# Tencent/PocketFlow

Hardware: NVIDIA H100
Metric: images_per_sec_compression_aware_training_step (higher is better)
Workload: dtype f32

## Files before the change

pocketflow_b200/csrc/pf_nn.cu:

```cuda
#include <cstdlib>
#include <numeric>

#include "pf_common.cuh"

namespace {

constexpr int NT = 256;
constexpr int kColTile = 256;

struct ColTile {
  int c0, tc, nvec, nty, tx, ty;
  __device__ ColTile(int C) {
    c0 = blockIdx.x * kColTile;
    tc = min(kColTile, C - c0);
    nvec = tc >> 2;
    nty = NT / nvec;
    tx = threadIdx.x % nvec;
    ty = threadIdx.x / nvec;
  }
};

template <bool RANGE>
__global__ void __launch_bounds__(NT)
bn_stats_partial_kernel(const float* __restrict__ x, int M, int C, int rows_per_split,
                        float* __restrict__ part ) {
  __shared__ float sh[RANGE ? 4 : 2][NT * 4];
  constexpr int NF = RANGE ? 5 : 3;
  const ColTile t(C);
  const int r0 = blockIdx.y * rows_per_split;
  const int r1 = min(M, r0 + rows_per_split);
  const int col = t.c0 + t.tx * 4;
  float4 K = make_float4(0.f, 0.f, 0.f, 0.f), s1 = K, s2 = K;
  float4 mn = make_float4(INFINITY, INFINITY, INFINITY, INFINITY), mx = make_float4(-INFINITY, -INFINITY, -INFINITY, -INFINITY);
  if (t.ty < t.nty) {
    K = __ldg(reinterpret_cast<const float4*>(x + (size_t)r0 * C + col));
    auto acc = [&](const float4 v) {
      if (RANGE) {
        mn.x = fminf(mn.x, v.x); mn.y = fminf(mn.y, v.y); mn.z = fminf(mn.z, v.z); mn.w = fminf(mn.w, v.w);
        mx.x = fmaxf(mx.x, v.x); mx.y = fmaxf(mx.y, v.y); mx.z = fmaxf(mx.z, v.z); mx.w = fmaxf(mx.w, v.w);
      }
      const float dx = v.x - K.x, dy = v.y - K.y, dz = v.z - K.z, dw = v.w - K.w;
      s1.x += dx; s1.y += dy; s1.z += dz; s1.w += dw;
      s2.x = fmaf(dx, dx, s2.x); s2.y = fmaf(dy, dy, s2.y); s2.z = fmaf(dz, dz, s2.z); s2.w = fmaf(dw, dw, s2.w);
    };
    int r = r0 + t.ty;
    for (; r + 3 * t.nty < r1; r += 4 * t.nty) {
      const float4 v0 = pf_ld_stream(x + (size_t)r * C + col);
      const float4 v1 = pf_ld_stream(x + (size_t)(r + t.nty) * C + col);
      const float4 v2 = pf_ld_stream(x + (size_t)(r + 2 * t.nty) * C + col);
      const float4 v3 = pf_ld_stream(x + (size_t)(r + 3 * t.nty) * C + col);
      acc(v0); acc(v1); acc(v2); acc(v3);
    }
    for (; r < r1; r += t.nty) acc(pf_ld_stream(x + (size_t)r * C + col));
    float* a = &sh[0][(t.ty * t.nvec + t.tx) * 4];
    float* b = &sh[1][(t.ty * t.nvec + t.tx) * 4];
    a[0] = s1.x; a[1] = s1.y; a[2] = s1.z; a[3] = s1.w;
    b[0] = s2.x; b[1] = s2.y; b[2] = s2.z; b[3] = s2.w;
    if (RANGE) {
      float* lo = &sh[RANGE ? 2 : 0][(t.ty * t.nvec + t.tx) * 4];
      float* hi = &sh[RANGE ? 3 : 0][(t.ty * t.nvec + t.tx) * 4];
      lo[0] = mn.x; lo[1] = mn.y; lo[2] = mn.z; lo[3] = mn.w;
      hi[0] = mx.x; hi[1] = mx.y; hi[2] = mx.z; hi[3] = mx.w;
    }
  }
  __syncthreads();
  for (int c = threadIdx.x; c < t.tc; c += NT) {
    float a = 0.f, b = 0.f, lo = INFINITY, hi = -INFINITY;
    for (int y = 0; y < t.nty; ++y) {
      a += sh[0][(y * t.nvec + (c >> 2)) * 4 + (c & 3)];
      b += sh[1][(y * t.nvec + (c >> 2)) * 4 + (c & 3)];
      if (RANGE) {
        lo = fminf(lo, sh[RANGE ? 2 : 0][(y * t.nvec + (c >> 2)) * 4 + (c & 3)]);
        hi = fmaxf(hi, sh[RANGE ? 3 : 0][(y * t.nvec + (c >> 2)) * 4 + (c & 3)]);
      }
    }
    float* p = part + (size_t)blockIdx.y * NF * C;
    p[t.c0 + c] = __ldg(x + (size_t)r0 * C + t.c0 + c);
    p[C + t.c0 + c] = a;
    p[2 * C + t.c0 + c] = b;
    if (RANGE) {
      p[3 * C + t.c0 + c] = lo;
      p[4 * C + t.c0 + c] = hi;
    }
  }
}

constexpr int kFinalWarps = 4;
__global__ void __launch_bounds__(NT)
bn_stats_final_kernel(const float* __restrict__ part, int M, int C, int splits, int rows_per_split,
                      float eps, float momentum, float* __restrict__ mean, float* __restrict__ var,
                      float* __restrict__ rstd, float* __restrict__ mov_mean, float* __restrict__ mov_var,
                      int nf, const float* __restrict__ gamma, const float* __restrict__ beta, int act,
                      uint32_t* __restrict__ minmax_enc) {
  constexpr int CPB = NT / 32 / kFinalWarps;
  __shared__ double sh1[NT / 32], sh2[NT / 32];
  __shared__ float shlo[NT / 32], shhi[NT / 32];
  const int lane = threadIdx.x & 31, warp = threadIdx.x >> 5;
  const int cl = warp / kFinalWarps, sub = warp % kFinalWarps;
  const int c = blockIdx.x * CPB + cl;
  double S1 = 0.0, S2 = 0.0;
  float xlo = INFINITY, xhi = -INFINITY;
  const double K0 = c < C ? (double)part[c] : 0.0;
  if (c < C) {
    for (int s = sub * 32 + lane; s < splits; s += 32 * kFinalWarps) {
      const int r0 = s * rows_per_split;
      const double n = (double)(min(M, r0 + rows_per_split) - r0);
      const float* p = part + (size_t)s * nf * C;
      const double d = (double)p[c] - K0, s1 = p[C + c], s2 = p[2 * C + c];
      S1 += s1 + n * d;
      S2 += s2 + 2.0 * d * s1 + n * d * d;
      if (nf == 5) {
        xlo = fminf(xlo, p[3 * C + c]);
        xhi = fmaxf(xhi, p[4 * C + c]);
      }
    }
  }
// ... 110 lines not shown
      const float4 mu = __ldg(reinterpret_cast<const float4*>(mean + c));
      float4 rs = __ldg(reinterpret_cast<const float4*>(rstd + c));
      if (var_eps >= 0.f) {
        rs.x = __frsqrt_rn(__fadd_rn(rs.x, var_eps)); rs.y = __frsqrt_rn(__fadd_rn(rs.y, var_eps));
        rs.z = __frsqrt_rn(__fadd_rn(rs.z, var_eps)); rs.w = __frsqrt_rn(__fadd_rn(rs.w, var_eps));
      }
      const float4 ga = __ldg(reinterpret_cast<const float4*>(gamma + c));
      const float4 be = __ldg(reinterpret_cast<const float4*>(beta + c));
      apply4(pf_ld_stream(x + (i << 2)), mu, rs, ga, be, i);
      c += step;
      if (c >= (uint32_t)C) c -= (uint32_t)C;
    }
  }
  if (minmax_enc) {
    mn = pf_warp_min(mn);
    mx = pf_warp_max(mx);
    const int lane = threadIdx.x & 31, wid = threadIdx.x >> 5;
    if (lane == 0) { s_mn[wid] = mn; s_mx[wid] = mx; }
    __syncthreads();
    if (wid == 0) {
      mn = lane < NT / 32 ? s_mn[lane] : INFINITY;
      mx = lane < NT / 32 ? s_mx[lane] : -INFINITY;
      mn = pf_warp_min(mn);
      mx = pf_warp_max(mx);
      if (lane == 0 && mn <= mx) {
        atomicMin(minmax_enc, pf_enc(mn));
        atomicMax(minmax_enc + 1, pf_enc(mx));
      }
    }
  }
}

template <bool LEVELS_ONLY>
__global__ void __launch_bounds__(NT)
bn_apply_levels_kernel(const float* __restrict__ x, int64_t total, int C, int cshift, const float* __restrict__ mean,
                       const float* __restrict__ rstd, const float* __restrict__ gamma, const float* __restrict__ beta,
                       int act, float* __restrict__ y, void* __restrict__ p0, void* __restrict__ p1,
                       const uint32_t* __restrict__ q_range, int q_bits, pf_tc_act_hdr* __restrict__ hdr,
                       float* __restrict__ csum, int nseg) {
  const float qmn = pf_dec(__ldg(q_range)), qmx = pf_dec(__ldg(q_range + 1));
  const float q_alpha = __fadd_rn(__fsub_rn(qmx, qmn), 1e-10f), q_beta = qmn;
  const float q_k = pf_uq_kf(q_bits), q_ra = __frcp_rn(q_alpha), q_rk = __frcp_rn(q_k);
  const bool lev = q_bits <= 8 && q_beta == 0.f;
  if (blockIdx.x == 0 && threadIdx.x == 0) {
    hdr->scale = lev ? __fdiv_rn(q_alpha, q_k) : 1.f;
    hdr->nplanes = lev ? 1 : 2;
  }
  const int lane = threadIdx.x & 31;
  const int L = min(C >> 2, 32);
  const int64_t nvec = total >> 2;
  const int64_t stride = (int64_t)gridDim.x * NT;
  const int64_t first = (int64_t)blockIdx.x * NT + threadIdx.x;
  const uint32_t c = (uint32_t)((first << 2) & (int64_t)(C - 1));
  const float4 mu = __ldg(reinterpret_cast<const float4*>(mean + c));
  const float4 rs = __ldg(reinterpret_cast<const float4*>(rstd + c));
  const float4 ga = __ldg(reinterpret_cast<const float4*>(gamma + c));
  const float4 be = __ldg(reinterpret_cast<const float4*>(beta + c));
  auto emit = [&](float4 v, int64_t i, bool valid) {
    float4 lv;
    if (LEVELS_ONLY && lev) {
      lv.x = pf_quant_level(pf_bn_act(v.x, mu.x, rs.x, ga.x, be.x, act), q_alpha, q_beta, q_k, q_ra);
      lv.y = pf_quant_level(pf_bn_act(v.y, mu.y, rs.y, ga.y, be.y, act), q_alpha, q_beta, q_k, q_ra);
      lv.z = pf_quant_level(pf_bn_act(v.z, mu.z, rs.z, ga.z, be.z, act), q_alpha, q_beta, q_k, q_ra);
      lv.w = pf_quant_level(pf_bn_act(v.w, mu.w, rs.w, ga.w, be.w, act), q_alpha, q_beta, q_k, q_ra);
    } else {
      v.x = pf_fake_quant_lv(pf_bn_act(v.x, mu.x, rs.x, ga.x, be.x, act), q_alpha, q_beta, q_k, q_ra, q_rk, lv.x);
      v.y = pf_fake_quant_lv(pf_bn_act(v.y, mu.y, rs.y, ga.y, be.y, act), q_alpha, q_beta, q_k, q_ra, q_rk, lv.y);
// ... 181 lines not shown
  const float q_alpha = __fadd_rn(__fsub_rn(qmx, qmn), 1e-10f);
  const float q_k = pf_uq_kf(q_bits), q_ra = __frcp_rn(q_alpha);
  if (blockIdx.x == 0 && threadIdx.x == 0) {
    hdr->scale = qmn == 0.f ? __fdiv_rn(q_alpha, q_k) : 1.f;
    hdr->nplanes = qmn == 0.f ? 1 : 0;
  }
  const int64_t wbase = first - (lane >> 3);
  for (int64_t i = first; wbase + (i - first) < items; i += stride) {
    float part = 0.f;
    if (i < items && cok) {
      float y[16];
      load_bn(i, y);
      uint32_t w[4];
#pragma unroll
      for (int v = 0; v < 4; ++v) {
        const float l0 = pf_quant_level(y[4 * v], q_alpha, qmn, q_k, q_ra);
        const float l1 = pf_quant_level(y[4 * v + 1], q_alpha, qmn, q_k, q_ra);
        const float l2 = pf_quant_level(y[4 * v + 2], q_alpha, qmn, q_k, q_ra);
        const float l3 = pf_quant_level(y[4 * v + 3], q_alpha, qmn, q_k, q_ra);
        w[v] = (uint32_t)l0 | ((uint32_t)l1 << 8) | ((uint32_t)l2 << 16) | ((uint32_t)l3 << 24);
        part += (l0 + l1) + (l2 + l3);
      }
      uint2* dst = reinterpret_cast<uint2*>(levels + (i / nseg) * C + c0);
      dst[0] = make_uint2(w[0], w[1]);
      dst[1] = make_uint2(w[2], w[3]);
    }
    part += __shfl_xor_sync(0xffffffffu, part, 4);
    part += __shfl_xor_sync(0xffffffffu, part, 2);
    part += __shfl_xor_sync(0xffffffffu, part, 1);
    if (i < items && sub == 0) csum[i] = part;
  }
}

__global__ void __launch_bounds__(NT)
bn_bwd_partial_kernel(const float* __restrict__ dy, const float* __restrict__ x, int M, int C,
                      int rows_per_split, const float* __restrict__ mean, const float* __restrict__ rstd,
                      const float* __restrict__ gamma, const float* __restrict__ beta, int act,
                      float* __restrict__ part ) {
  __shared__ float sh[2][NT * 4];
  const ColTile t(C);
  const int r0 = blockIdx.y * rows_per_split;
  const int r1 = min(M, r0 + rows_per_split);
  const int col = t.c0 + t.tx * 4;
  float a[4] = {0.f, 0.f, 0.f, 0.f}, b[4] = {0.f, 0.f, 0.f, 0.f};
  if (t.ty < t.nty) {
    const float4 mu4 = __ldg(reinterpret_cast<const float4*>(mean + col));
    const float4 rs4 = __ldg(reinterpret_cast<const float4*>(rstd + col));
    const float4 ga4 = __ldg(reinterpret_cast<const float4*>(gamma + col));
    const float4 be4 = __ldg(reinterpret_cast<const float4*>(beta + col));
    const float mu[4] = {mu4.x, mu4.y, mu4.z, mu4.w}, rs[4] = {rs4.x, rs4.y, rs4.z, rs4.w};
    const float ga[4] = {ga4.x, ga4.y, ga4.z, ga4.w}, be[4] = {be4.x, be4.y, be4.z, be4.w};
    for (int r = r0 + t.ty; r < r1; r += t.nty) {
      const float4 d4 = pf_ld_stream(dy + (size_t)r * C + col);
      const float4 x4 = pf_ld_stream(x + (size_t)r * C + col);
      const float d[4] = {d4.x, d4.y, d4.z, d4.w}, xv[4] = {x4.x, x4.y, x4.z, x4.w};
#pragma unroll
      for (int j = 0; j < 4; ++j) {
        const float xh = __fmul_rn(__fsub_rn(xv[j], mu[j]), rs[j]);
        float dz = d[j];
        if (act) {
          const float z = __fadd_rn(__fmul_rn(xh, ga[j]), be[j]);
          if (!(z > 0.f) || (act == 2 && !(z < 6.f))) dz = 0.f;
        }
        a[j] += dz;
        b[j] = fmaf(dz, xh, b[j]);
      }
    }
    float* pa = &sh[0][(t.ty * t.nvec + t.tx) * 4];
    float* pb = &sh[1][(t.ty * t.nvec + t.tx) * 4];
#pragma unroll
    for (int j = 0; j < 4; ++j) { pa[j] = a[j]; pb[j] = b[j]; }
  }
  __syncthreads();
  for (int c = threadIdx.x; c < t.tc; c += NT) {
    float sa = 0.f, sb = 0.f;
    for (int y = 0; y < t.nty; ++y) {
      sa += sh[0][(y * t.nvec + (c >> 2)) * 4 + (c & 3)];
      sb += sh[1][(y * t.nvec + (c >> 2)) * 4 + (c & 3)];
    }
    float* p = part + (size_t)blockIdx.y * 2 * C;
    p[t.c0 + c] = sa;
    p[C + t.c0 + c] = sb;
  }
}

__global__ void __launch_bounds__(NT)
bn_bwd_final_kernel(const float* __restrict__ part, int C, int splits, float* __restrict__ dgamma,
                    float* __restrict__ dbeta) {
  constexpr int CPB = NT / 32 / kFinalWarps;
  __shared__ double sha[NT / 32], shb[NT / 32];
  const int lane = threadIdx.x & 31, warp = threadIdx.x >> 5;
  const int cl = warp / kFinalWarps, sub = warp % kFinalWarps;
  const int c = blockIdx.x * CPB + cl;
  double sa = 0.0, sb = 0.0;
  if (c < C) {
    for (int s = sub * 32 + lane; s < splits; s += 32 * kFinalWarps) {
      sa += part[(size_t)s * 2 * C + c];
      sb += part[(size_t)s * 2 * C + C + c];
    }
  }
#pragma unroll
  for (int o = 16; o > 0; o >>= 1) {
    sa += __shfl_down_sync(0xffffffffu, sa, o);
    sb += __shfl_down_sync(0xffffffffu, sb, o);
  }
  if (lane == 0) { sha[warp] = sa; shb[warp] = sb; }
  __syncthreads();
  if (c < C && sub == 0 && lane == 0) {
    for (int w = 1; w < kFinalWarps; ++w) { sa += sha[warp + w]; sb += shb[warp + w]; }
    dbeta[c] = (float)sa;
    dgamma[c] = (float)sb;
  }
}

__global__ void __launch_bounds__(NT)
bn_bwd_apply_kernel(const float* __restrict__ dy, const float* __restrict__ x, int64_t total, int C,
                    float inv_m, const float* __restrict__ mean, const float* __restrict__ rstd,
                    const float* __restrict__ gamma, const float* __restrict__ beta,
                    const float* __restrict__ dgamma, const float* __restrict__ dbeta, int act,
                    int accumulate, float* __restrict__ dx, void* __restrict__ dx_hi, void* __restrict__ dx_lo) {
  const int64_t nvec = total >> 2;
  const int64_t stride = (int64_t)gridDim.x * NT;
  int64_t i = (int64_t)blockIdx.x * NT + threadIdx.x;
  uint32_t c = (uint32_t)((i << 2) % (uint32_t)C);
  const uint32_t step = (uint32_t)((stride << 2) % (uint32_t)C);
  auto one = [&](const float4 d4, const float4 x4, const float4 mu4, const float4 rs4, const float4 ga4,
                 const float4 be4, const float4 dg4, const float4 db4, int64_t idx) {
    const float d[4] = {d4.x, d4.y, d4.z, d4.w}, xv[4] = {x4.x, x4.y, x4.z, x4.w};
    const float mu[4] = {mu4.x, mu4.y, mu4.z, mu4.w}, rs[4] = {rs4.x, rs4.y, rs4.z, rs4.w};
    const float ga[4] = {ga4.x, ga4.y, ga4.z, ga4.w}, be[4] = {be4.x, be4.y, be4.z, be4.w};
    const float dg[4] = {dg4.x, dg4.y, dg4.z, dg4.w}, db[4] = {db4.x, db4.y, db4.z, db4.w};
    float o[4];
#pragma unroll
    for (int j = 0; j < 4; ++j) {
      const float xh = __fmul_rn(__fsub_rn(xv[j], mu[j]), rs[j]);
      float dz = d[j];
      if (act) {
        const float z = __fadd_rn(__fmul_rn(xh, ga[j]), be[j]);
        if (!(z > 0.f) || (act == 2 && !(z < 6.f))) dz = 0.f;
      }
      o[j] = ga[j] * rs[j] * (dz - db[j] * inv_m - xh * dg[j] * inv_m);
    }
    float4 r = make_float4(o[0], o[1], o[2], o[3]);
    if (accumulate) {
      const float4 old = *reinterpret_cast<const float4*>(dx + (idx << 2));
      r.x += old.x; r.y += old.y; r.z += old.z; r.w += old.w;
    }
    if (dx) pf_st_stream(dx + (idx << 2), r);
    if (dx_hi) pf_st_planes4(dx_hi, dx_lo, idx << 2, r);
  };
  if (step == 0) {
    const float4 mu4 = __ldg(reinterpret_cast<const float4*>(mean + c)), rs4 = __ldg(reinterpret_cast<const float4*>(rstd + c));
    const float4 ga4 = __ldg(reinterpret_cast<const float4*>(gamma + c)), be4 = __ldg(reinterpret_cast<const float4*>(beta + c));
    const float4 dg4 = __ldg(reinterpret_cast<const float4*>(dgamma + c)), db4 = __ldg(reinterpret_cast<const float4*>(dbeta + c));
    for (; i + stride < nvec; i += 2 * stride) {
      const float4 d0 = pf_ld_stream(dy + (i << 2)), x0 = pf_ld_stream(x + (i << 2));
      const float4 d1 = pf_ld_stream(dy + ((i + stride) << 2)), x1 = pf_ld_stream(x + ((i + stride) << 2));
      one(d0, x0, mu4, rs4, ga4, be4, dg4, db4, i);
      one(d1, x1, mu4, rs4, ga4, be4, dg4, db4, i + stride);
    }
    for (; i < nvec; i += stride)
      one(pf_ld_stream(dy + (i << 2)), pf_ld_stream(x + (i << 2)), mu4, rs4, ga4, be4, dg4, db4, i);
  } else {
    for (; i < nvec; i += stride) {
      one(pf_ld_stream(dy + (i << 2)), pf_ld_stream(x + (i << 2)), __ldg(reinterpret_cast<const float4*>(mean + c)),
          __ldg(reinterpret_cast<const float4*>(rstd + c)), __ldg(reinterpret_cast<const float4*>(gamma + c)),
          __ldg(reinterpret_cast<const float4*>(beta + c)), __ldg(reinterpret_cast<const float4*>(dgamma + c)),
          __ldg(reinterpret_cast<const float4*>(dbeta + c)), i);
      c += step;
      if (c >= (uint32_t)C) c -= (uint32_t)C;
    }
  }
}

__global__ void __launch_bounds__(NT)
add_kernel(const float* __restrict__ a, const float* __restrict__ b, int64_t n, int accumulate,
           float* __restrict__ out) {
  const int64_t nvec = n >> 2;
  const int64_t stride = (int64_t)gridDim.x * NT;
  for (int64_t i = (int64_t)blockIdx.x * NT + threadIdx.x; i < nvec; i += stride) {
    float4 v = pf_ld4(a + (i << 2));
    if (b) {
      const float4 w = pf_ld4(b + (i << 2));
      v.x = __fadd_rn(v.x, w.x); v.y = __fadd_rn(v.y, w.y); v.z = __fadd_rn(v.z, w.z); v.w = __fadd_rn(v.w, w.w);
    }
    if (accumulate) {
      const float4 o = pf_ld4(out + (i << 2));
      v.x += o.x; v.y += o.y; v.z += o.z; v.w += o.w;
    }
    pf_st_stream(out + (i << 2), v);
  }
  if (blockIdx.x == 0 && threadIdx.x < (n & 3)) {
    const int64_t j = (nvec << 2) + threadIdx.x;
    float v = a[j] + (b ? b[j] : 0.f);
    out[j] = accumulate ? out[j] + v : v;
  }
}

// ... 217 lines not shown
__global__ void __launch_bounds__(NT)
softmax_fwd_kernel(const float* __restrict__ x, int n, int k, float* __restrict__ y) {
  const int lane = threadIdx.x & 31;
  const int row = blockIdx.x * (NT / 32) + (threadIdx.x >> 5);
  if (row >= n) return;
  const float* r = x + (size_t)row * k;
  float m = -INFINITY;
  for (int j = lane; j < k; j += 32) m = fmaxf(m, r[j]);
  m = pf_warp_max(m);
  float s = 0.f;
  for (int j = lane; j < k; j += 32) s += expf(r[j] - m);
  s = pf_warp_sum(s);
  for (int j = lane; j < k; j += 32) y[(size_t)row * k + j] = __fdiv_rn(expf(r[j] - m), s);
}
__global__ void __launch_bounds__(NT)
softmax_bwd_kernel(const float* __restrict__ dy, const float* __restrict__ y, int n, int k,
                   float* __restrict__ dx) {
  const int lane = threadIdx.x & 31;
  const int row = blockIdx.x * (NT / 32) + (threadIdx.x >> 5);
  if (row >= n) return;
  float dot = 0.f;
  for (int j = lane; j < k; j += 32) dot += dy[(size_t)row * k + j] * y[(size_t)row * k + j];
  dot = pf_warp_sum(dot);
  for (int j = lane; j < k; j += 32) {
    const size_t o = (size_t)row * k + j;
    dx[o] = (dy[o] - dot) * y[o];
  }
}

inline int bn_grid_cap() {
  const char* v = getenv("PF_BN_GRIDCAP");
  return (v && *v) ? atoi(v) : 8;
}
inline unsigned chan_grid(int64_t nvec, int C) {
  int64_t want = (nvec + NT - 1) / NT;
  const int64_t cap = (int64_t)PF_NUM_SMS * bn_grid_cap();
  if (want > cap) want = cap;
  if (want < 1) want = 1;
  const int c4 = C >> 2;
  int64_t mult = 1;
  while ((mult * NT) % c4 != 0 && mult < 64) mult <<= 1;
  if ((mult * NT) % c4 == 0) want = (want + mult - 1) / mult * mult;
  return (unsigned)want;
}

inline unsigned ew_grid(int64_t work_items) {
  int64_t want = (work_items + NT - 1) / NT;
  const int64_t cap = (int64_t)PF_NUM_SMS * 8;
  if (want < 1) want = 1;
  return (unsigned)(want < cap ? want : cap);
}

inline int bn_splits(int M, int C, int* rows_per_split) {
  const int col_tiles = (C + kColTile - 1) / kColTile;
  int splits = (8 * PF_NUM_SMS + col_tiles - 1) / col_tiles;
  const int max_by_rows = (M + 63) / 64;
  if (splits > max_by_rows) splits = max_by_rows;
  if (splits > PF_BN_MAX_SPLITS) splits = PF_BN_MAX_SPLITS;
  if (splits < 1) splits = 1;
  int rps = (M + splits - 1) / splits;
  *rows_per_split = rps;
  return (M + rps - 1) / rps;
}

__global__ void __launch_bounds__(NT)
fold_diag_blocks_kernel(const float* __restrict__ src, int g, int m, int n, float* __restrict__ dst) {
  const int i = blockIdx.x * NT + threadIdx.x;
  if (i >= m * n) return;
  const int r = i / n, c = i - r * n;
  float acc = 0.f;
  for (int b = 0; b < g; ++b) acc += src[(size_t)(b * m + r) * (g * n) + b * n + c];
  dst[i] = acc;
}
}

extern "C" {

int pf_bn_train_stats_range(const float* x_dev, int64_t m, int c, float eps, float momentum, float* mean_dev,
                            float* var_dev, float* rstd_dev, float* moving_mean_dev, float* moving_var_dev,
                            const float* gamma_dev, const float* beta_dev, int act, uint32_t* minmax_enc_dev,
                            float* ws_dev, void* stream) {
  PF_REQUIRE(m > 0 && c > 0 && m < (1ll << 31), "pf_bn_train_stats: bad shape");
  PF_REQUIRE((c & 3) == 0, "pf_bn_train_stats: C must be a multiple of 4 (got %d)", c);
  PF_REQUIRE(x_dev && mean_dev && var_dev && rstd_dev && ws_dev, "pf_bn_train_stats: null pointer");
  PF_REQUIRE((moving_mean_dev == nullptr) == (moving_var_dev == nullptr), "pf_bn_train_stats: moving stats come in pairs");
  PF_REQUIRE(minmax_enc_dev == nullptr || (gamma_dev && beta_dev && act >= 0 && act <= 2),
             "pf_bn_train_stats_range: the output range needs gamma, beta and act in {0,1,2}");
  int rps;
  const int splits = bn_splits((int)m, c, &rps);
  dim3 grid((c + kColTile - 1) / kColTile, splits);
  cudaStream_t st = (cudaStream_t)stream;
  const int nf = minmax_enc_dev ? 5 : 3;
  if (minmax_enc_dev) bn_stats_partial_kernel<true><<<grid, NT, 0, st>>>(x_dev, (int)m, c, rps, ws_dev);
  else bn_stats_partial_kernel<false><<<grid, NT, 0, st>>>(x_dev, (int)m, c, rps, ws_dev);
  PF_CHECK_LAUNCH("pf_bn_train_stats/partial");
  constexpr int kCPB = NT / 32 / kFinalWarps;
  bn_stats_final_kernel<<<(c + kCPB - 1) / kCPB, NT, 0, st>>>(ws_dev, (int)m, c, splits, rps, eps, momentum, mean_dev,
                                                         var_dev, rstd_dev, moving_mean_dev, moving_var_dev, nf, gamma_dev,
                                                         beta_dev, act, minmax_enc_dev);
  PF_CHECK_LAUNCH("pf_bn_train_stats/final");
  return PF_OK;
}

int pf_bn_train_stats(const float* x_dev, int64_t m, int c, float eps, float momentum, float* mean_dev,
                      float* var_dev, float* rstd_dev, float* moving_mean_dev, float* moving_var_dev,
                      float* ws_dev, void* stream) {
  return pf_bn_train_stats_range(x_dev, m, c, eps, momentum, mean_dev, var_dev, rstd_dev, moving_mean_dev, moving_var_dev,
                                 nullptr, nullptr, 0, nullptr, ws_dev, stream);
}

int pf_bn_eval_prepare(const float* moving_var_dev, int c, float eps, float* rstd_dev, void* stream) {
  PF_REQUIRE(c > 0 && moving_var_dev && rstd_dev, "pf_bn_eval_prepare: bad arguments");
  bn_eval_prepare_kernel<<<(c + NT - 1) / NT, NT, 0, (cudaStream_t)stream>>>(moving_var_dev, c, eps, rstd_dev);
  PF_CHECK_LAUNCH("pf_bn_eval_prepare");
  return PF_OK;
}

static int bn_apply_impl(const float* x_dev, int64_t m, int c, const float* mean_dev, const float* rstd_dev,
                         const float* gamma_dev, const float* beta_dev, int act, float* y_dev, void* y_hi_dev,
                         void* y_lo_dev, uint32_t* minmax_enc_dev, const uint32_t* q_range_dev, int q_bits, void* stream,
                         float var_eps = -1.f, const float* res_dev = nullptr) {
  PF_REQUIRE(m > 0 && c > 0 && (c & 3) == 0, "pf_bn_apply: bad shape (C must be a multiple of 4)");
  PF_REQUIRE(act >= 0 && act <= 2, "pf_bn_apply: act must be 0 (none), 1 (relu) or 2 (relu6)");
  PF_REQUIRE(x_dev && mean_dev && rstd_dev && gamma_dev && beta_dev, "pf_bn_apply: null pointer");
  PF_REQUIRE(y_dev || y_hi_dev, "pf_bn_apply: no output");
  PF_REQUIRE((y_hi_dev == nullptr) == (y_lo_dev == nullptr), "pf_bn_apply: planes come in pairs");
  PF_REQUIRE((((uintptr_t)y_hi_dev | (uintptr_t)y_lo_dev) & 7) == 0, "pf_bn_apply: planes must be 8-byte aligned");
// ... 20 lines not shown

int pf_bn_apply_eval(const float* x_dev, int64_t m, int c, const float* moving_mean_dev, const float* moving_var_dev,
                     float eps, const float* gamma_dev, const float* beta_dev, int act, float* y_dev, void* y_hi_dev,
                     void* y_lo_dev, uint32_t* minmax_enc_dev, void* stream) {
  PF_REQUIRE(eps >= 0.f, "pf_bn_apply_eval: eps < 0");
  return bn_apply_impl(x_dev, m, c, moving_mean_dev, moving_var_dev, gamma_dev, beta_dev, act, y_dev, y_hi_dev, y_lo_dev,
                       minmax_enc_dev, nullptr, 0, stream, eps);
}

int pf_bn_apply_quant(const float* x_dev, int64_t m, int c, const float* mean_dev, const float* rstd_dev,
                      const float* gamma_dev, const float* beta_dev, int act, const uint32_t* range_enc_dev, int bits,
                      float* y_dev, void* y_hi_dev, void* y_lo_dev, void* stream) {
  PF_REQUIRE(range_enc_dev != nullptr, "pf_bn_apply_quant: null range");
  PF_REQUIRE(bits >= 1 && bits <= 32, "pf_bn_apply_quant: bits must be in [1, 32]");
  return bn_apply_impl(x_dev, m, c, mean_dev, rstd_dev, gamma_dev, beta_dev, act, y_dev, y_hi_dev, y_lo_dev, nullptr,
                       range_enc_dev, bits, stream);
}

int pf_bn_apply_quant_levels(const float* x_dev, int64_t m, int c, const float* mean_dev, const float* rstd_dev,
                             const float* gamma_dev, const float* beta_dev, int act, const uint32_t* range_enc_dev,
                             int bits, float* y_dev, void* plane0_dev, void* plane1_dev, pf_tc_act_hdr* hdr_dev,
                             float* csum_dev, void* stream) {
  PF_REQUIRE(m > 0 && c >= 16 && (c & (c - 1)) == 0, "pf_bn_apply_quant_levels: C must be a power of two >= 16 (got %d)", c);
  PF_REQUIRE(act >= 0 && act <= 2, "pf_bn_apply_quant_levels: act must be 0 (none), 1 (relu) or 2 (relu6)");
  PF_REQUIRE(bits >= 1 && bits <= 32, "pf_bn_apply_quant_levels: bits must be in [1, 32]");
  PF_REQUIRE(x_dev && mean_dev && rstd_dev && gamma_dev && beta_dev && range_enc_dev && plane0_dev && plane1_dev && hdr_dev &&
                 csum_dev, "pf_bn_apply_quant_levels: null pointer");
  PF_REQUIRE((((uintptr_t)plane0_dev | (uintptr_t)plane1_dev | (uintptr_t)hdr_dev) & 7) == 0,
             "pf_bn_apply_quant_levels: planes / header must be 8-byte aligned");
  const int64_t total = m * c;
  int cshift = 0;
  while ((1 << cshift) < c) ++cshift;
  const int nseg = (c + 127) / 128;
  unsigned grid = chan_grid(total >> 2, c);
  PF_REQUIRE(((int64_t)grid * NT) % (c >> 2) == 0, "pf_bn_apply_quant_levels: C = %d too large for the channel-stationary grid", c);
  if (y_dev == nullptr && bits <= 8)
    bn_apply_levels_kernel<true><<<grid, NT, 0, (cudaStream_t)stream>>>(x_dev, total, c, cshift, mean_dev, rstd_dev, gamma_dev,
                                                                       beta_dev, act, nullptr, plane0_dev, plane1_dev,
                                                                       range_enc_dev, bits, hdr_dev, csum_dev, nseg);
  else
    bn_apply_levels_kernel<false><<<grid, NT, 0, (cudaStream_t)stream>>>(x_dev, total, c, cshift, mean_dev, rstd_dev, gamma_dev,
                                                                        beta_dev, act, y_dev, plane0_dev, plane1_dev,
                                                                        range_enc_dev, bits, hdr_dev, csum_dev, nseg);
  PF_CHECK_LAUNCH("pf_bn_apply_quant_levels");
  return PF_OK;
}

int pf_bn_eval_levels_u8(const float* x_dev, int64_t m, int c, const float* moving_mean_dev, const float* moving_var_dev,
                         float eps, const float* gamma_dev, const float* beta_dev, int act, int bits,
                         uint32_t* range_enc_dev, int have_range, void* levels_dev, pf_tc_act_hdr* hdr_dev,
                         float* csum_dev, void* stream) {
  const char* who = "pf_bn_eval_levels_u8";
  PF_REQUIRE(m > 0 && c >= 16 && c % 16 == 0, "%s: C must be a multiple of 16 (got %d)", who, c);
  PF_REQUIRE(act >= 0 && act <= 2, "%s: act must be 0 (none), 1 (relu) or 2 (relu6)", who);
  PF_REQUIRE(bits >= 1 && bits <= 8, "%s: u8 levels need 1..8 bits", who);
  PF_REQUIRE(eps >= 0.f, "%s: eps < 0", who);
  PF_REQUIRE(x_dev && moving_mean_dev && moving_var_dev && gamma_dev && beta_dev && range_enc_dev && levels_dev && hdr_dev &&
                 csum_dev, "%s: null pointer", who);
  PF_REQUIRE((((uintptr_t)x_dev | (uintptr_t)moving_mean_dev | (uintptr_t)moving_var_dev | (uintptr_t)gamma_dev |
               (uintptr_t)beta_dev) & 15) == 0 && (((uintptr_t)levels_dev | (uintptr_t)hdr_dev) & 7) == 0,
             "%s: fp32 tensors must be 16-byte aligned, levels / header 8-byte aligned", who);
  const int64_t total = m * c;
  const int nseg = (c + 127) / 128;
  cudaStream_t st = (cudaStream_t)stream;
  uint8_t* lv = reinterpret_cast<uint8_t*>(levels_dev);
  if (c & (c - 1)) {
    const int64_t items = m * nseg;
// ... 44 lines not shown

int pf_bn_apply_add_eval(const float* x_dev, int64_t m, int c, const float* moving_mean_dev, const float* moving_var_dev,
                         float eps, const float* gamma_dev, const float* beta_dev, const float* res_dev, float* y_dev,
                         void* y_hi_dev, void* y_lo_dev, void* stream) {
  PF_REQUIRE(eps >= 0.f, "pf_bn_apply_add_eval: eps < 0");
  PF_REQUIRE(res_dev != nullptr, "pf_bn_apply_add_eval: null residual");
  PF_REQUIRE((((uintptr_t)res_dev | (uintptr_t)x_dev | (uintptr_t)y_dev) & 15) == 0,
             "pf_bn_apply_add_eval: fp32 tensors must be 16-byte aligned");
  return bn_apply_impl(x_dev, m, c, moving_mean_dev, moving_var_dev, gamma_dev, beta_dev, 0, y_dev, y_hi_dev, y_lo_dev, nullptr,
                       nullptr, 0, stream, eps, res_dev);
}

int pf_bn_apply(const float* x_dev, int64_t m, int c, const float* mean_dev, const float* rstd_dev,
                const float* gamma_dev, const float* beta_dev, int act, float* y_dev,
                uint32_t* minmax_enc_dev, void* stream) {
  PF_REQUIRE(y_dev != nullptr, "pf_bn_apply: null pointer");
  return pf_bn_apply_planes(x_dev, m, c, mean_dev, rstd_dev, gamma_dev, beta_dev, act, y_dev, nullptr, nullptr,
                            minmax_enc_dev, stream);
}

int pf_bn_bwd_planes(const float* dy_dev, const float* x_dev, int64_t m, int c, const float* mean_dev,
                     const float* rstd_dev, const float* gamma_dev, const float* beta_dev, int act,
                     float* dgamma_dev, float* dbeta_dev, float* dx_dev, int accumulate, void* dx_hi_dev,
                     void* dx_lo_dev, float* ws_dev, void* stream) {
  PF_REQUIRE(m > 0 && c > 0 && (c & 3) == 0 && m < (1ll << 31), "pf_bn_bwd: bad shape (C must be a multiple of 4)");
  PF_REQUIRE(dy_dev && x_dev && mean_dev && rstd_dev && gamma_dev && beta_dev && dgamma_dev && dbeta_dev && ws_dev,
             "pf_bn_bwd: null pointer");
  PF_REQUIRE(dx_dev || dx_hi_dev, "pf_bn_bwd: no output");
  PF_REQUIRE((dx_hi_dev == nullptr) == (dx_lo_dev == nullptr), "pf_bn_bwd: planes come in pairs");
  PF_REQUIRE(!accumulate || dx_dev, "pf_bn_bwd: accumulate needs the fp32 dx");
  PF_REQUIRE((((uintptr_t)dx_hi_dev | (uintptr_t)dx_lo_dev) & 7) == 0, "pf_bn_bwd: planes must be 8-byte aligned");
  int rps;
  const int splits = bn_splits((int)m, c, &rps);
  dim3 grid((c + kColTile - 1) / kColTile, splits);
  cudaStream_t st = (cudaStream_t)stream;
  bn_bwd_partial_kernel<<<grid, NT, 0, st>>>(dy_dev, x_dev, (int)m, c, rps, mean_dev, rstd_dev, gamma_dev, beta_dev,
                                            act, ws_dev);
  PF_CHECK_LAUNCH("pf_bn_bwd/partial");
  bn_bwd_final_kernel<<<(c + NT / 32 / kFinalWarps - 1) / (NT / 32 / kFinalWarps), NT, 0, st>>>(ws_dev, c, splits, dgamma_dev, dbeta_dev);
  PF_CHECK_LAUNCH("pf_bn_bwd/final");
  const int64_t total = m * c;
  bn_bwd_apply_kernel<<<chan_grid(total >> 2, c), NT, 0, st>>>(dy_dev, x_dev, total, c, 1.f / (float)m, mean_dev, rstd_dev,
                                                        gamma_dev, beta_dev, dgamma_dev, dbeta_dev, act, accumulate,
                                                        dx_dev, dx_hi_dev, dx_lo_dev);
  PF_CHECK_LAUNCH("pf_bn_bwd/apply");
  return PF_OK;
}

int pf_bn_bwd(const float* dy_dev, const float* x_dev, int64_t m, int c, const float* mean_dev,
              const float* rstd_dev, const float* gamma_dev, const float* beta_dev, int act,
              float* dgamma_dev, float* dbeta_dev, float* dx_dev, int accumulate, float* ws_dev,
              void* stream) {
  PF_REQUIRE(dx_dev != nullptr, "pf_bn_bwd: null pointer");
  return pf_bn_bwd_planes(dy_dev, x_dev, m, c, mean_dev, rstd_dev, gamma_dev, beta_dev, act, dgamma_dev, dbeta_dev,
                          dx_dev, accumulate, nullptr, nullptr, ws_dev, stream);
}

int pf_fold_diag_blocks(const float* src_dev, int g, int m, int n, float* dst_dev, void* stream) {
  PF_REQUIRE(g >= 1 && m >= 1 && n >= 1 && (int64_t)m * n < (1ll << 30), "pf_fold_diag_blocks: bad shape");
  PF_REQUIRE(src_dev && dst_dev, "pf_fold_diag_blocks: null pointer");
  fold_diag_blocks_kernel<<<(m * n + NT - 1) / NT, NT, 0, (cudaStream_t)stream>>>(src_dev, g, m, n, dst_dev);
  PF_CHECK_LAUNCH("pf_fold_diag_blocks");
  return PF_OK;
}

int pf_add(const float* a_dev, const float* b_dev, int64_t n, int accumulate, float* out_dev, void* stream) {
  PF_REQUIRE(n >= 0, "pf_add: n < 0");
  if (n == 0) return PF_OK;
  PF_REQUIRE(a_dev && out_dev, "pf_add: null pointer");
  PF_REQUIRE((((uintptr_t)a_dev | (uintptr_t)b_dev | (uintptr_t)out_dev) & 15) == 0, "pf_add: 16-byte alignment required");
  add_kernel<<<ew_grid(n >> 2), NT, 0, (cudaStream_t)stream>>>(a_dev, b_dev, n, accumulate, out_dev);
  PF_CHECK_LAUNCH("pf_add");
  return PF_OK;
}

// ... 87 lines not shown
```

Baseline: 2749.

## Cap batchnorm grids to SM residency and make partial kernels loop over splits

The BN stats and backward partial kernels become grid-stride over row splits, with the grid capped to a per-SM CTA target and splits walked in reverse. Launch-bound minimum-block hints are added, and the backward partial loop is unrolled four rows at a time. The backward apply kernel goes from two to four vectors per iteration and loads the old dx before computing. The aim is to cut tail and wave-quantisation effects and expose more memory-level parallelism, at the cost of register pressure from the launch bounds and fewer CTAs for small shapes.

```diff
diff --git a/pocketflow_b200/csrc/pf_nn.cu b/pocketflow_b200/csrc/pf_nn.cu
--- a/pocketflow_b200/csrc/pf_nn.cu
+++ b/pocketflow_b200/csrc/pf_nn.cu
@@ -1,3 +1,4 @@
+#include <algorithm>
 #include <cstdlib>
 #include <numeric>
 
@@ -7,6 +8,10 @@
 
 constexpr int NT = 256;
 constexpr int kColTile = 256;
+constexpr int kStatsCtasPerSm = 4;
+constexpr int kBwdCtasPerSm = 3;
+constexpr int kBwdApplyCtasPerSm = 2;
+constexpr int kApplyLevelsCtasPerSm = 4;
 
 struct ColTile {
   int c0, tc, nvec, nty, tx, ty;
@@ -21,67 +26,71 @@
 };
 
 template <bool RANGE>
-__global__ void __launch_bounds__(NT)
-bn_stats_partial_kernel(const float* __restrict__ x, int M, int C, int rows_per_split,
+__global__ void __launch_bounds__(NT, kStatsCtasPerSm)
+bn_stats_partial_kernel(const float* __restrict__ x, int M, int C, int rows_per_split, int splits,
                         float* __restrict__ part ) {
   __shared__ float sh[RANGE ? 4 : 2][NT * 4];
   constexpr int NF = RANGE ? 5 : 3;
   const ColTile t(C);
-  const int r0 = blockIdx.y * rows_per_split;
-  const int r1 = min(M, r0 + rows_per_split);
   const int col = t.c0 + t.tx * 4;
-  float4 K = make_float4(0.f, 0.f, 0.f, 0.f), s1 = K, s2 = K;
-  float4 mn = make_float4(INFINITY, INFINITY, INFINITY, INFINITY), mx = make_float4(-INFINITY, -INFINITY, -INFINITY, -INFINITY);
-  if (t.ty < t.nty) {
-    K = __ldg(reinterpret_cast<const float4*>(x + (size_t)r0 * C + col));
-    auto acc = [&](const float4 v) {
+  for (int k = blockIdx.y; k < splits; k += gridDim.y) {
+    const int split = splits - 1 - k;
+    const int r0 = split * rows_per_split;
+    const int r1 = min(M, r0 + rows_per_split);
+    float4 K = make_float4(0.f, 0.f, 0.f, 0.f), s1 = K, s2 = K;
+    float4 mn = make_float4(INFINITY, INFINITY, INFINITY, INFINITY), mx = make_float4(-INFINITY, -INFINITY, -INFINITY, -INFINITY);
+    if (t.ty < t.nty) {
+      K = __ldg(reinterpret_cast<const float4*>(x + (size_t)r0 * C + col));
+      auto acc = [&](const float4 v) {
+        if (RANGE) {
+          mn.x = fminf(mn.x, v.x); mn.y = fminf(mn.y, v.y); mn.z = fminf(mn.z, v.z); mn.w = fminf(mn.w, v.w);
+          mx.x = fmaxf(mx.x, v.x); mx.y = fmaxf(mx.y, v.y); mx.z = fmaxf(mx.z, v.z); mx.w = fmaxf(mx.w, v.w);
+        }
+        const float dx = v.x - K.x, dy = v.y - K.y, dz = v.z - K.z, dw = v.w - K.w;
+        s1.x += dx; s1.y += dy; s1.z += dz; s1.w += dw;
+        s2.x = fmaf(dx, dx, s2.x); s2.y = fmaf(dy, dy, s2.y); s2.z = fmaf(dz, dz, s2.z); s2.w = fmaf(dw, dw, s2.w);
+      };
+      int r = r0 + t.ty;
+      for (; r + 3 * t.nty < r1; r += 4 * t.nty) {
+        const float4 v0 = pf_ld_stream(x + (size_t)r * C + col);
+        const float4 v1 = pf_ld_stream(x + (size_t)(r + t.nty) * C + col);
+        const float4 v2 = pf_ld_stream(x + (size_t)(r + 2 * t.nty) * C + col);
+        const float4 v3 = pf_ld_stream(x + (size_t)(r + 3 * t.nty) * C + col);
+        acc(v0); acc(v1); acc(v2); acc(v3);
+      }
+      for (; r < r1; r += t.nty) acc(pf_ld_stream(x + (size_t)r * C + col));
+      float* a = &sh[0][(t.ty * t.nvec + t.tx) * 4];
+      float* b = &sh[1][(t.ty * t.nvec + t.tx) * 4];
+      a[0] = s1.x; a[1] = s1.y; a[2] = s1.z; a[3] = s1.w;
+      b[0] = s2.x; b[1] = s2.y; b[2] = s2.z; b[3] = s2.w;
       if (RANGE) {
-        mn.x = fminf(mn.x, v.x); mn.y = fminf(mn.y, v.y); mn.z = fminf(mn.z, v.z); mn.w = fminf(mn.w, v.w);
-        mx.x = fmaxf(mx.x, v.x); mx.y = fmaxf(mx.y, v.y); mx.z = fmaxf(mx.z, v.z); mx.w = fmaxf(mx.w, v.w);
-      }
-      const float dx = v.x - K.x, dy = v.y - K.y, dz = v.z - K.z, dw = v.w - K.w;
-      s1.x += dx; s1.y += dy; s1.z += dz; s1.w += dw;
-      s2.x = fmaf(dx, dx, s2.x); s2.y = fmaf(dy, dy, s2.y); s2.z = fmaf(dz, dz, s2.z); s2.w = fmaf(dw, dw, s2.w);
-    };
-    int r = r0 + t.ty;
-    for (; r + 3 * t.nty < r1; r += 4 * t.nty) {
-      const float4 v0 = pf_ld_stream(x + (size_t)r * C + col);
-      const float4 v1 = pf_ld_stream(x + (size_t)(r + t.nty) * C + col);
-      const float4 v2 = pf_ld_stream(x + (size_t)(r + 2 * t.nty) * C + col);
-      const float4 v3 = pf_ld_stream(x + (size_t)(r + 3 * t.nty) * C + col);
-      acc(v0); acc(v1); acc(v2); acc(v3);
-    }
-    for (; r < r1; r += t.nty) acc(pf_ld_stream(x + (size_t)r * C + col));
-    float* a = &sh[0][(t.ty * t.nvec + t.tx) * 4];
-    float* b = &sh[1][(t.ty * t.nvec + t.tx) * 4];
-    a[0] = s1.x; a[1] = s1.y; a[2] = s1.z; a[3] = s1.w;
-    b[0] = s2.x; b[1] = s2.y; b[2] = s2.z; b[3] = s2.w;
-    if (RANGE) {
-      float* lo = &sh[RANGE ? 2 : 0][(t.ty * t.nvec + t.tx) * 4];
-      float* hi = &sh[RANGE ? 3 : 0][(t.ty * t.nvec + t.tx) * 4];
-      lo[0] = mn.x; lo[1] = mn.y; lo[2] = mn.z; lo[3] = mn.w;
-      hi[0] = mx.x; hi[1] = mx.y; hi[2] = mx.z; hi[3] = mx.w;
-    }
-  }
-  __syncthreads();
-  for (int c = threadIdx.x; c < t.tc; c += NT) {
-    float a = 0.f, b = 0.f, lo = INFINITY, hi = -INFINITY;
-    for (int y = 0; y < t.nty; ++y) {
-      a += sh[0][(y * t.nvec + (c >> 2)) * 4 + (c & 3)];
-      b += sh[1][(y * t.nvec + (c >> 2)) * 4 + (c & 3)];
+        float* lo = &sh[RANGE ? 2 : 0][(t.ty * t.nvec + t.tx) * 4];
+        float* hi = &sh[RANGE ? 3 : 0][(t.ty * t.nvec + t.tx) * 4];
+        lo[0] = mn.x; lo[1] = mn.y; lo[2] = mn.z; lo[3] = mn.w;
+        hi[0] = mx.x; hi[1] = mx.y; hi[2] = mx.z; hi[3] = mx.w;
+      }
+    }
+    __syncthreads();
+    for (int c = threadIdx.x; c < t.tc; c += NT) {
+      float a = 0.f, b = 0.f, lo = INFINITY, hi = -INFINITY;
+      for (int y = 0; y < t.nty; ++y) {
+        a += sh[0][(y * t.nvec + (c >> 2)) * 4 + (c & 3)];
+        b += sh[1][(y * t.nvec + (c >> 2)) * 4 + (c & 3)];
+        if (RANGE) {
+          lo = fminf(lo, sh[RANGE ? 2 : 0][(y * t.nvec + (c >> 2)) * 4 + (c & 3)]);
+          hi = fmaxf(hi, sh[RANGE ? 3 : 0][(y * t.nvec + (c >> 2)) * 4 + (c & 3)]);
+        }
+      }
+      float* p = part + (size_t)split * NF * C;
+      p[t.c0 + c] = __ldg(x + (size_t)r0 * C + t.c0 + c);
+      p[C + t.c0 + c] = a;
+      p[2 * C + t.c0 + c] = b;
       if (RANGE) {
-        lo = fminf(lo, sh[RANGE ? 2 : 0][(y * t.nvec + (c >> 2)) * 4 + (c & 3)]);
-        hi = fmaxf(hi, sh[RANGE ? 3 : 0][(y * t.nvec + (c >> 2)) * 4 + (c & 3)]);
-      }
-    }
-    float* p = part + (size_t)blockIdx.y * NF * C;
-    p[t.c0 + c] = __ldg(x + (size_t)r0 * C + t.c0 + c);
-    p[C + t.c0 + c] = a;
-    p[2 * C + t.c0 + c] = b;
-    if (RANGE) {
-      p[3 * C + t.c0 + c] = lo;
-      p[4 * C + t.c0 + c] = hi;
-    }
+        p[3 * C + t.c0 + c] = lo;
+        p[4 * C + t.c0 + c] = hi;
+      }
+    }
+    __syncthreads();
   }
 }
 
@@ -258,7 +267,7 @@
 }
 
 template <bool LEVELS_ONLY>
-__global__ void __launch_bounds__(NT)
+__global__ void __launch_bounds__(NT, kApplyLevelsCtasPerSm)
 bn_apply_levels_kernel(const float* __restrict__ x, int64_t total, int C, int cshift, const float* __restrict__ mean,
                        const float* __restrict__ rstd, const float* __restrict__ gamma, const float* __restrict__ beta,
                        int act, float* __restrict__ y, void* __restrict__ p0, void* __restrict__ p1,
@@ -506,55 +515,74 @@
   }
 }
 
-__global__ void __launch_bounds__(NT)
+__global__ void __launch_bounds__(NT, kBwdCtasPerSm)
 bn_bwd_partial_kernel(const float* __restrict__ dy, const float* __restrict__ x, int M, int C,
-                      int rows_per_split, const float* __restrict__ mean, const float* __restrict__ rstd,
+                      int rows_per_split, int splits, const float* __restrict__ mean, const float* __restrict__ rstd,
                       const float* __restrict__ gamma, const float* __restrict__ beta, int act,
                       float* __restrict__ part ) {
   __shared__ float sh[2][NT * 4];
   const ColTile t(C);
-  const int r0 = blockIdx.y * rows_per_split;
-  const int r1 = min(M, r0 + rows_per_split);
   const int col = t.c0 + t.tx * 4;
-  float a[4] = {0.f, 0.f, 0.f, 0.f}, b[4] = {0.f, 0.f, 0.f, 0.f};
+  float mu[4], rs[4], ga[4], be[4];
   if (t.ty < t.nty) {
     const float4 mu4 = __ldg(reinterpret_cast<const float4*>(mean + col));
     const float4 rs4 = __ldg(reinterpret_cast<const float4*>(rstd + col));
     const float4 ga4 = __ldg(reinterpret_cast<const float4*>(gamma + col));
     const float4 be4 = __ldg(reinterpret_cast<const float4*>(beta + col));
-    const float mu[4] = {mu4.x, mu4.y, mu4.z, mu4.w}, rs[4] = {rs4.x, rs4.y, rs4.z, rs4.w};
-    const float ga[4] = {ga4.x, ga4.y, ga4.z, ga4.w}, be[4] = {be4.x, be4.y, be4.z, be4.w};
-    for (int r = r0 + t.ty; r < r1; r += t.nty) {
-      const float4 d4 = pf_ld_stream(dy + (size_t)r * C + col);
-      const float4 x4 = pf_ld_stream(x + (size_t)r * C + col);
-      const float d[4] = {d4.x, d4.y, d4.z, d4.w}, xv[4] = {x4.x, x4.y, x4.z, x4.w};
-#pragma unroll
-      for (int j = 0; j < 4; ++j) {
-        const float xh = __fmul_rn(__fsub_rn(xv[j], mu[j]), rs[j]);
-        float dz = d[j];
-        if (act) {
-          const float z = __fadd_rn(__fmul_rn(xh, ga[j]), be[j]);
-          if (!(z > 0.f) || (act == 2 && !(z < 6.f))) dz = 0.f;
+    mu[0] = mu4.x; mu[1] = mu4.y; mu[2] = mu4.z; mu[3] = mu4.w;
+    rs[0] = rs4.x; rs[1] = rs4.y; rs[2] = rs4.z; rs[3] = rs4.w;
+    ga[0] = ga4.x; ga[1] = ga4.y; ga[2] = ga4.z; ga[3] = ga4.w;
+    be[0] = be4.x; be[1] = be4.y; be[2] = be4.z; be[3] = be4.w;
+  }
+  for (int k = blockIdx.y; k < splits; k += gridDim.y) {
+    const int split = splits - 1 - k;
+    const int r0 = split * rows_per_split;
+    const int r1 = min(M, r0 + rows_per_split);
+    float a[4] = {0.f, 0.f, 0.f, 0.f}, b[4] = {0.f, 0.f, 0.f, 0.f};
+    if (t.ty < t.nty) {
+      auto acc = [&](const float4 d4, const float4 x4) {
+        const float d[4] = {d4.x, d4.y, d4.z, d4.w}, xv[4] = {x4.x, x4.y, x4.z, x4.w};
+#pragma unroll
+        for (int j = 0; j < 4; ++j) {
+          const float xh = __fmul_rn(__fsub_rn(xv[j], mu[j]), rs[j]);
+          float dz = d[j];
+          if (act) {
+            const float z = __fadd_rn(__fmul_rn(xh, ga[j]), be[j]);
+            if (!(z > 0.f) || (act == 2 && !(z < 6.f))) dz = 0.f;
+          }
+          a[j] += dz;
+          b[j] = fmaf(dz, xh, b[j]);
         }
-        a[j] += dz;
-        b[j] = fmaf(dz, xh, b[j]);
-      }
-    }
-    float* pa = &sh[0][(t.ty * t.nvec + t.tx) * 4];
-    float* pb = &sh[1][(t.ty * t.nvec + t.tx) * 4];
-#pragma unroll
-    for (int j = 0; j < 4; ++j) { pa[j] = a[j]; pb[j] = b[j]; }
-  }
-  __syncthreads();
-  for (int c = threadIdx.x; c < t.tc; c += NT) {
-    float sa = 0.f, sb = 0.f;
-    for (int y = 0; y < t.nty; ++y) {
-      sa += sh[0][(y * t.nvec + (c >> 2)) * 4 + (c & 3)];
-      sb += sh[1][(y * t.nvec + (c >> 2)) * 4 + (c & 3)];
-    }
-    float* p = part + (size_t)blockIdx.y * 2 * C;
-    p[t.c0 + c] = sa;
-    p[C + t.c0 + c] = sb;
+      };
+      int r = r0 + t.ty;
+      for (; r + 3 * t.nty < r1; r += 4 * t.nty) {
+        const float* pd = dy + (size_t)r * C + col;
+        const float* px = x + (size_t)r * C + col;
+        const size_t rs1 = (size_t)t.nty * C;
+        const float4 d0 = pf_ld_stream(pd), x0 = pf_ld_stream(px);
+        const float4 d1 = pf_ld_stream(pd + rs1), x1 = pf_ld_stream(px + rs1);
+        const float4 d2 = pf_ld_stream(pd + 2 * rs1), x2 = pf_ld_stream(px + 2 * rs1);
+        const float4 d3 = pf_ld_stream(pd + 3 * rs1), x3 = pf_ld_stream(px + 3 * rs1);
+        acc(d0, x0); acc(d1, x1); acc(d2, x2); acc(d3, x3);
+      }
+      for (; r < r1; r += t.nty) acc(pf_ld_stream(dy + (size_t)r * C + col), pf_ld_stream(x + (size_t)r * C + col));
+      float* pa = &sh[0][(t.ty * t.nvec + t.tx) * 4];
+      float* pb = &sh[1][(t.ty * t.nvec + t.tx) * 4];
+#pragma unroll
+      for (int j = 0; j < 4; ++j) { pa[j] = a[j]; pb[j] = b[j]; }
+    }
+    __syncthreads();
+    for (int c = threadIdx.x; c < t.tc; c += NT) {
+      float sa = 0.f, sb = 0.f;
+      for (int y = 0; y < t.nty; ++y) {
+        sa += sh[0][(y * t.nvec + (c >> 2)) * 4 + (c & 3)];
+        sb += sh[1][(y * t.nvec + (c >> 2)) * 4 + (c & 3)];
+      }
+      float* p = part + (size_t)split * 2 * C;
+      p[t.c0 + c] = sa;
+      p[C + t.c0 + c] = sb;
+    }
+    __syncthreads();
   }
 }
 
@@ -587,7 +615,7 @@
   }
 }
 
-__global__ void __launch_bounds__(NT)
+__global__ void __launch_bounds__(NT, kBwdApplyCtasPerSm)
 bn_bwd_apply_kernel(const float* __restrict__ dy, const float* __restrict__ x, int64_t total, int C,
                     float inv_m, const float* __restrict__ mean, const float* __restrict__ rstd,
                     const float* __restrict__ gamma, const float* __restrict__ beta,
@@ -598,8 +626,8 @@
   int64_t i = (int64_t)blockIdx.x * NT + threadIdx.x;
   uint32_t c = (uint32_t)((i << 2) % (uint32_t)C);
   const uint32_t step = (uint32_t)((stride << 2) % (uint32_t)C);
-  auto one = [&](const float4 d4, const float4 x4, const float4 mu4, const float4 rs4, const float4 ga4,
-                 const float4 be4, const float4 dg4, const float4 db4, int64_t idx) {
+  auto one = [&](const float4 d4, const float4 x4, const float4 old, const float4 mu4, const float4 rs4,
+                 const float4 ga4, const float4 be4, const float4 dg4, const float4 db4, int64_t idx) {
     const float d[4] = {d4.x, d4.y, d4.z, d4.w}, xv[4] = {x4.x, x4.y, x4.z, x4.w};
     const float mu[4] = {mu4.x, mu4.y, mu4.z, mu4.w}, rs[4] = {rs4.x, rs4.y, rs4.z, rs4.w};
     const float ga[4] = {ga4.x, ga4.y, ga4.z, ga4.w}, be[4] = {be4.x, be4.y, be4.z, be4.w};
@@ -617,27 +645,35 @@
     }
     float4 r = make_float4(o[0], o[1], o[2], o[3]);
     if (accumulate) {
-      const float4 old = *reinterpret_cast<const float4*>(dx + (idx << 2));
       r.x += old.x; r.y += old.y; r.z += old.z; r.w += old.w;
     }
     if (dx) pf_st_stream(dx + (idx << 2), r);
     if (dx_hi) pf_st_planes4(dx_hi, dx_lo, idx << 2, r);
+  };
+  auto old_dx = [&](int64_t idx) {
+    return accumulate ? *reinterpret_cast<const float4*>(dx + (idx << 2)) : make_float4(0.f, 0.f, 0.f, 0.f);
   };
   if (step == 0) {
     const float4 mu4 = __ldg(reinterpret_cast<const float4*>(mean + c)), rs4 = __ldg(reinterpret_cast<const float4*>(rstd + c));
     const float4 ga4 = __ldg(reinterpret_cast<const float4*>(gamma + c)), be4 = __ldg(reinterpret_cast<const float4*>(beta + c));
     const float4 dg4 = __ldg(reinterpret_cast<const float4*>(dgamma + c)), db4 = __ldg(reinterpret_cast<const float4*>(dbeta + c));
-    for (; i + stride < nvec; i += 2 * stride) {
+    for (; i + 3 * stride < nvec; i += 4 * stride) {
+      const int64_t i1 = i + stride, i2 = i1 + stride, i3 = i2 + stride;
       const float4 d0 = pf_ld_stream(dy + (i << 2)), x0 = pf_ld_stream(x + (i << 2));
-      const float4 d1 = pf_ld_stream(dy + ((i + stride) << 2)), x1 = pf_ld_stream(x + ((i + stride) << 2));
-      one(d0, x0, mu4, rs4, ga4, be4, dg4, db4, i);
-      one(d1, x1, mu4, rs4, ga4, be4, dg4, db4, i + stride);
+      const float4 d1 = pf_ld_stream(dy + (i1 << 2)), x1 = pf_ld_stream(x + (i1 << 2));
+      const float4 d2 = pf_ld_stream(dy + (i2 << 2)), x2 = pf_ld_stream(x + (i2 << 2));
+      const float4 d3 = pf_ld_stream(dy + (i3 << 2)), x3 = pf_ld_stream(x + (i3 << 2));
+      const float4 o0 = old_dx(i), o1 = old_dx(i1), o2 = old_dx(i2), o3 = old_dx(i3);
+      one(d0, x0, o0, mu4, rs4, ga4, be4, dg4, db4, i);
+      one(d1, x1, o1, mu4, rs4, ga4, be4, dg4, db4, i1);
+      one(d2, x2, o2, mu4, rs4, ga4, be4, dg4, db4, i2);
+      one(d3, x3, o3, mu4, rs4, ga4, be4, dg4, db4, i3);
     }
     for (; i < nvec; i += stride)
-      one(pf_ld_stream(dy + (i << 2)), pf_ld_stream(x + (i << 2)), mu4, rs4, ga4, be4, dg4, db4, i);
+      one(pf_ld_stream(dy + (i << 2)), pf_ld_stream(x + (i << 2)), old_dx(i), mu4, rs4, ga4, be4, dg4, db4, i);
   } else {
     for (; i < nvec; i += stride) {
-      one(pf_ld_stream(dy + (i << 2)), pf_ld_stream(x + (i << 2)), __ldg(reinterpret_cast<const float4*>(mean + c)),
+      one(pf_ld_stream(dy + (i << 2)), pf_ld_stream(x + (i << 2)), old_dx(i), __ldg(reinterpret_cast<const float4*>(mean + c)),
           __ldg(reinterpret_cast<const float4*>(rstd + c)), __ldg(reinterpret_cast<const float4*>(gamma + c)),
           __ldg(reinterpret_cast<const float4*>(beta + c)), __ldg(reinterpret_cast<const float4*>(dgamma + c)),
           __ldg(reinterpret_cast<const float4*>(dbeta + c)), i);
@@ -921,9 +957,9 @@
   const char* v = getenv("PF_BN_GRIDCAP");
   return (v && *v) ? atoi(v) : 8;
 }
-inline unsigned chan_grid(int64_t nvec, int C) {
+inline unsigned chan_grid(int64_t nvec, int C, int ctas_per_sm = bn_grid_cap()) {
   int64_t want = (nvec + NT - 1) / NT;
-  const int64_t cap = (int64_t)PF_NUM_SMS * bn_grid_cap();
+  const int64_t cap = (int64_t)PF_NUM_SMS * ctas_per_sm;
   if (want > cap) want = cap;
   if (want < 1) want = 1;
   const int c4 = C >> 2;
@@ -950,6 +986,13 @@
   int rps = (M + splits - 1) / splits;
   *rows_per_split = rps;
   return (M + rps - 1) / rps;
+}
+
+inline dim3 partial_grid(int C, int splits, int ctas_per_sm) {
+  const int col_tiles = (C + kColTile - 1) / kColTile;
+  const int cap = std::max(1, ctas_per_sm * PF_NUM_SMS / col_tiles);
+  const int per_cta = (splits + cap - 1) / cap;
+  return dim3(col_tiles, (splits + per_cta - 1) / per_cta);
 }
 
 __global__ void __launch_bounds__(NT)
@@ -977,11 +1020,11 @@
              "pf_bn_train_stats_range: the output range needs gamma, beta and act in {0,1,2}");
   int rps;
   const int splits = bn_splits((int)m, c, &rps);
-  dim3 grid((c + kColTile - 1) / kColTile, splits);
+  const dim3 grid = partial_grid(c, splits, kStatsCtasPerSm);
   cudaStream_t st = (cudaStream_t)stream;
   const int nf = minmax_enc_dev ? 5 : 3;
-  if (minmax_enc_dev) bn_stats_partial_kernel<true><<<grid, NT, 0, st>>>(x_dev, (int)m, c, rps, ws_dev);
-  else bn_stats_partial_kernel<false><<<grid, NT, 0, st>>>(x_dev, (int)m, c, rps, ws_dev);
+  if (minmax_enc_dev) bn_stats_partial_kernel<true><<<grid, NT, 0, st>>>(x_dev, (int)m, c, rps, splits, ws_dev);
+  else bn_stats_partial_kernel<false><<<grid, NT, 0, st>>>(x_dev, (int)m, c, rps, splits, ws_dev);
   PF_CHECK_LAUNCH("pf_bn_train_stats/partial");
   constexpr int kCPB = NT / 32 / kFinalWarps;
   bn_stats_final_kernel<<<(c + kCPB - 1) / kCPB, NT, 0, st>>>(ws_dev, (int)m, c, splits, rps, eps, momentum, mean_dev,
@@ -1068,7 +1111,7 @@
   int cshift = 0;
   while ((1 << cshift) < c) ++cshift;
   const int nseg = (c + 127) / 128;
-  unsigned grid = chan_grid(total >> 2, c);
+  unsigned grid = chan_grid(total >> 2, c, kApplyLevelsCtasPerSm);
   PF_REQUIRE(((int64_t)grid * NT) % (c >> 2) == 0, "pf_bn_apply_quant_levels: C = %d too large for the channel-stationary grid", c);
   if (y_dev == nullptr && bits <= 8)
     bn_apply_levels_kernel<true><<<grid, NT, 0, (cudaStream_t)stream>>>(x_dev, total, c, cshift, mean_dev, rstd_dev, gamma_dev,
@@ -1179,15 +1222,14 @@
   PF_REQUIRE((((uintptr_t)dx_hi_dev | (uintptr_t)dx_lo_dev) & 7) == 0, "pf_bn_bwd: planes must be 8-byte aligned");
   int rps;
   const int splits = bn_splits((int)m, c, &rps);
-  dim3 grid((c + kColTile - 1) / kColTile, splits);
   cudaStream_t st = (cudaStream_t)stream;
-  bn_bwd_partial_kernel<<<grid, NT, 0, st>>>(dy_dev, x_dev, (int)m, c, rps, mean_dev, rstd_dev, gamma_dev, beta_dev,
-                                            act, ws_dev);
+  bn_bwd_partial_kernel<<<partial_grid(c, splits, kBwdCtasPerSm), NT, 0, st>>>(dy_dev, x_dev, (int)m, c, rps, splits, mean_dev, rstd_dev,
+                                                               gamma_dev, beta_dev, act, ws_dev);
   PF_CHECK_LAUNCH("pf_bn_bwd/partial");
   bn_bwd_final_kernel<<<(c + NT / 32 / kFinalWarps - 1) / (NT / 32 / kFinalWarps), NT, 0, st>>>(ws_dev, c, splits, dgamma_dev, dbeta_dev);
   PF_CHECK_LAUNCH("pf_bn_bwd/final");
   const int64_t total = m * c;
-  bn_bwd_apply_kernel<<<chan_grid(total >> 2, c), NT, 0, st>>>(dy_dev, x_dev, total, c, 1.f / (float)m, mean_dev, rstd_dev,
+  bn_bwd_apply_kernel<<<chan_grid(total >> 2, c, kBwdApplyCtasPerSm), NT, 0, st>>>(dy_dev, x_dev, total, c, 1.f / (float)m, mean_dev, rstd_dev,
                                                         gamma_dev, beta_dev, dgamma_dev, dbeta_dev, act, accumulate,
                                                         dx_dev, dx_hi_dev, dx_lo_dev);
   PF_CHECK_LAUNCH("pf_bn_bwd/apply");
```

Result: no change. 2754 (median of 6 runs) (+0.2%).
